# vincentfung13/MINE

Measured on AMD Instinct MI355X. Metric: train imgs/sec (whole node) RealEstate10K 384x256 N=64, higher is better.
Workload: dtype bf16; 1 GPU; model=monodepth2-resnet50-mpi, global_batch=4, seq_len=64, parallelism=dp1, img_h=256, img_w=384, n_planes=64

## Files before the change

mine_amd/ops/csrc/bindings.hip:

```cpp

#include <torch/extension.h>
#include <ATen/hip/HIPContext.h>
#include <hip/hip_runtime.h>

#include <vector>

extern "C" {
void mine_src_composite_fwd(const float*, const float*, const float*,
                            const float*, float*, float*, float*, int, int,
                            int, int, int, int, hipStream_t);
void mine_src_composite_bwd(const float*, const float*, const float*,
                            const float*, const float*, const float*,
                            const float*, float*, int, int, int, int, int,
                            int, hipStream_t);
void mine_tgt_composite_fwd(const float*, const float*, const float*,
                            const float*, const float*, float*, float*,
                            float*, int, int, int, int, int, int,
                            hipStream_t);
void mine_tgt_composite_bwd(const float*, const float*, const float*,
                            const float*, const float*, const float*,
                            const float*, const float*, float*, float*,
                            int, int, int, int, int, int, int, hipStream_t);
void mine_conv_igemm_fwd(const void*, const void*, const float*, void*,
                         float*, int64_t, int, int, int, int, int, int, int,
// ... 130 lines not shown
  const at::ScalarType t = dtype.value_or(at::kBFloat16);
  TORCH_CHECK(is_16bit(t), who, ": output dtype must be bf16 or fp16");
  return t;
}

std::vector<at::Tensor> src_composite_fwd(at::Tensor mpi, at::Tensor depths,
                                          at::Tensor kinv, at::Tensor img,
                                          bool bg_inf, bool alpha) {
  CHECK_IN(mpi); CHECK_IN(depths); CHECK_IN(kinv);
  TORCH_CHECK(mpi.dim() == 5 && mpi.size(4) == 4, "mpi must be (B,S,H,W,4)");
  const int B = mpi.size(0), S = mpi.size(1), H = mpi.size(2), W = mpi.size(3);
  TORCH_CHECK(S <= 192, "S too large for the LDS geometry stage");
  const bool blend = img.numel() > 0;
  if (blend) {
    CHECK_IN(img);
    TORCH_CHECK(img.sizes() == at::IntArrayRef({B, H, W, 3}),
                "img must be (B,H,W,3)");
  }
  auto rgb = at::empty({B, 3, H, W}, mpi.options());
  auto depth = at::empty({B, 1, H, W}, mpi.options());
  auto mpi_blend = blend ? at::empty_like(mpi) : at::empty({0}, mpi.options());
  mine_src_composite_fwd(mpi.data_ptr<float>(), depths.data_ptr<float>(),
                         kinv.data_ptr<float>(), optr(img),
                         rgb.data_ptr<float>(), depth.data_ptr<float>(),
                         blend ? mpi_blend.data_ptr<float>() : nullptr,
                         B, S, H, W, bg_inf ? 1 : 0, alpha ? 1 : 0,
                         stream());
  return {rgb, depth, mpi_blend};
}

at::Tensor src_composite_bwd(at::Tensor mpi, at::Tensor depths,
                             at::Tensor kinv, at::Tensor img, bool bg_inf,
                             bool alpha, at::Tensor g_rgb,
                             at::Tensor g_depth, at::Tensor g_blend) {
  CHECK_IN(mpi);
  const int B = mpi.size(0), S = mpi.size(1), H = mpi.size(2), W = mpi.size(3);
  auto grad_mpi = at::empty_like(mpi);
  mine_src_composite_bwd(mpi.data_ptr<float>(), depths.data_ptr<float>(),
                         kinv.data_ptr<float>(), optr(img), optr(g_rgb),
                         optr(g_depth), optr(g_blend),
                         grad_mpi.data_ptr<float>(), B, S, H, W,
                         bg_inf ? 1 : 0, alpha ? 1 : 0, stream());
  return grad_mpi;
}

std::vector<at::Tensor> tgt_composite_fwd(at::Tensor mpi, at::Tensor hinv,
                                          at::Tensor m, at::Tensor tvec,
                                          at::Tensor depths, bool bg_inf,
                                          bool alpha) {
  CHECK_IN(mpi); CHECK_IN(hinv); CHECK_IN(m); CHECK_IN(tvec); CHECK_IN(depths);
  TORCH_CHECK(mpi.dim() == 5 && mpi.size(4) == 4, "mpi must be (B,S,H,W,4)");
  const int B = mpi.size(0), S = mpi.size(1), H = mpi.size(2), W = mpi.size(3);
  TORCH_CHECK(S <= 192, "S too large for the LDS geometry stage");
  TORCH_CHECK(hinv.sizes() == at::IntArrayRef({B, S, 3, 3}));
  auto rgb = at::empty({B, 3, H, W}, mpi.options());
  auto depth = at::empty({B, 1, H, W}, mpi.options());
  auto mask = at::empty({B, 1, H, W}, mpi.options());
  mine_tgt_composite_fwd(mpi.data_ptr<float>(), hinv.data_ptr<float>(),
                         m.data_ptr<float>(), tvec.data_ptr<float>(),
                         depths.data_ptr<float>(), rgb.data_ptr<float>(),
                         depth.data_ptr<float>(), mask.data_ptr<float>(),
                         B, S, H, W, bg_inf ? 1 : 0, alpha ? 1 : 0,
                         stream());
  return {rgb, depth, mask};
}

at::Tensor tgt_composite_bwd(at::Tensor mpi, at::Tensor hinv, at::Tensor hfwd,
                             at::Tensor m, at::Tensor tvec, at::Tensor depths,
                             bool bg_inf, bool alpha, at::Tensor g_rgb,
                             at::Tensor g_depth, int64_t mode) {
  CHECK_IN(mpi);
  const int B = mpi.size(0), S = mpi.size(1), H = mpi.size(2), W = mpi.size(3);
  auto grad_mpi = at::zeros_like(mpi);
  at::Tensor payload;
  float* pay_ptr = nullptr;
  if (mode == 1) {
    TORCH_CHECK(hfwd.numel() == (int64_t)B * S * 9, "hfwd required in gather mode");
    payload = at::zeros_like(mpi);
    pay_ptr = payload.data_ptr<float>();
  }
  mine_tgt_composite_bwd(mpi.data_ptr<float>(), hinv.data_ptr<float>(),
                         mode == 1 ? hfwd.data_ptr<float>() : nullptr,
                         m.data_ptr<float>(), tvec.data_ptr<float>(),
                         depths.data_ptr<float>(), optr(g_rgb), optr(g_depth),
                         grad_mpi.data_ptr<float>(), pay_ptr, B, S, H, W,
                         bg_inf ? 1 : 0, (int)mode, alpha ? 1 : 0, stream());
  return grad_mpi;
}


at::Tensor eav2_fwd(at::Tensor disp, at::Tensor img, at::Tensor mean_d) {
  TORCH_CHECK(disp.is_cuda() && disp.is_contiguous() &&
              disp.scalar_type() == at::kFloat &&
              img.scalar_type() == at::kFloat);
  const int B = disp.size(0), H = disp.size(2), W = disp.size(3);
  auto out = at::zeros({2}, disp.options());
  mine_eav2_fwd(disp.data_ptr<float>(), img.data_ptr<float>(),
                mean_d.data_ptr<float>(), out.data_ptr<float>(), B, H, W,
                img.stride(0), img.stride(1), img.stride(2), img.stride(3),
                stream());
  return out;
}

at::Tensor eav2_bwd(at::Tensor disp, at::Tensor img, at::Tensor mean_d,
                    at::Tensor gl) {
  const int B = disp.size(0), H = disp.size(2), W = disp.size(3);
  auto g_d = at::empty({B, 1, H, W}, disp.options());
  auto Tb = at::zeros({B}, disp.options());
  auto grad = at::empty_like(disp);
  mine_eav2_bwd(disp.data_ptr<float>(), img.data_ptr<float>(),
                mean_d.data_ptr<float>(), g_d.data_ptr<float>(),
                Tb.data_ptr<float>(), gl.data_ptr<float>(),
                grad.data_ptr<float>(), B, H, W,
                img.stride(0), img.stride(1), img.stride(2), img.stride(3),
                stream());
  return grad;
}

at::Tensor pack_gather(at::Tensor w, at::Tensor lut,
                       c10::optional<at::ScalarType> dtype) {
  TORCH_CHECK(w.is_cuda() && w.is_contiguous() && lut.is_contiguous());
  TORCH_CHECK(lut.scalar_type() == at::kInt);
  TORCH_CHECK(w.scalar_type() == at::kFloat || is_16bit(w.scalar_type()),
              "pack_gather: weight must be f32, bf16 or fp16");
  const at::ScalarType ot = pack_dtype(dtype, "pack_gather");
  auto out = at::empty({lut.numel()}, w.options().dtype(ot));
  mine_pack_gather(w.data_ptr(), lut.data_ptr<int>(), out.data_ptr(),
                   lut.numel(), w_kind(w.scalar_type()),
                   ot == at::kHalf ? 1 : 0, stream());
  return out;
}
// ... 489 lines not shown
bool g_window_set = false;

void ensure_window() {
  if (g_window_set) return;
  double w[11], sum = 0.0;
  for (int i = 0; i < 11; ++i) {
    const double d = i - 5;
    w[i] = std::exp(-d * d / (2.0 * 1.5 * 1.5));
    sum += w[i];
  }
  float wf[11];
  for (int i = 0; i < 11; ++i) wf[i] = (float)(w[i] / sum);
  mine_ssim_set_window(wf);
  g_window_set = true;
}

std::vector<at::Tensor> ssim_fwd(at::Tensor img1, at::Tensor img2) {
  CHECK_IN(img1); CHECK_IN(img2);
  TORCH_CHECK(img1.dim() == 4 && img1.sizes() == img2.sizes());
  ensure_window();
  const int BC = img1.size(0) * img1.size(1);
  const int H = img1.size(2), W = img1.size(3);
  auto sum = at::zeros({1}, img1.options());
  mine_ssim_fwd(img1.data_ptr<float>(), img2.data_ptr<float>(),
                sum.data_ptr<float>(), BC, H, W, stream());
  return {(sum / (double)(BC * (int64_t)H * W)).squeeze(0)};
}

at::Tensor ssim_bwd(at::Tensor img1, at::Tensor img2, at::Tensor gscale) {
  CHECK_IN(img1); CHECK_IN(img2);
  ensure_window();
  const int BC = img1.size(0) * img1.size(1);
  const int H = img1.size(2), W = img1.size(3);
  auto F1 = at::empty_like(img1);
  auto F2 = at::empty_like(img1);
  auto F3 = at::empty_like(img1);
  auto grad1 = at::empty_like(img1);
  auto g = gscale.to(img1.options()).contiguous();
  mine_ssim_bwd(img1.data_ptr<float>(), img2.data_ptr<float>(),
                g.data_ptr<float>(), F1.data_ptr<float>(),
                F2.data_ptr<float>(), F3.data_ptr<float>(),
                grad1.data_ptr<float>(), BC, H, W, stream());
  return grad1;
}

}

PYBIND11_MODULE(TORCH_EXTENSION_NAME, mod) {
  mod.def("src_composite_fwd", &src_composite_fwd,
          "fused src-view MPI composite + RGB blend, forward");
  mod.def("src_composite_bwd", &src_composite_bwd);
  mod.def("tgt_composite_fwd", &tgt_composite_fwd,
          "fused plane-sweep warp + z-cull + composite, forward");
  mod.def("tgt_composite_bwd", &tgt_composite_bwd);
  mod.def("ssim_fwd", &ssim_fwd);
  mod.def("ssim_bwd", &ssim_bwd);
  mod.def("eav2_fwd", &eav2_fwd, "fused edge-aware smoothness v2 fwd");
  mod.def("eav2_bwd", &eav2_bwd, "fused edge-aware smoothness v2 bwd");
  namespace py = pybind11;
  mod.def("pack_gather", &pack_gather,
          "one-launch fragment pack through a device LUT", py::arg("w"),
          py::arg("lut"), py::arg("dtype") = py::none());
  mod.def("conv_igemm_fwd", &conv_igemm_fwd,
          "general igemm conv fwd / data-grad (coordinate-remapped)",
          py::arg("x_flat"), py::arg("wp"), py::arg("bias"), py::arg("M"),
          py::arg("P"), py::arg("Q"), py::arg("K"), py::arg("Hs"),
          py::arg("Ws"), py::arg("C"), py::arg("R"), py::arg("S"),
          py::arg("SA"), py::arg("SB"), py::arg("SD"), py::arg("SE"),
          py::arg("pad_mode"), py::arg("deterministic") = false);
  mod.def("conv_igemm_wrw", &conv_igemm_wrw,
          "general igemm conv weight-grad", py::arg("x_flat"),
          py::arg("gy_flat"), py::arg("M"), py::arg("P"), py::arg("Q"),
          py::arg("K"), py::arg("Hs"), py::arg("Ws"), py::arg("C"),
          py::arg("R"), py::arg("S"), py::arg("SA"), py::arg("SB"),
          py::arg("SD"), py::arg("SE"), py::arg("pad_mode"),
          py::arg("deterministic") = false);
  mod.def("upsample2x_fwd", &upsample2x_fwd,
          "nearest x2 upsample fwd, flat NHWC");
  mod.def("upsample2x_bwd", &upsample2x_bwd,
          "nearest x2 upsample bwd (4-child sum), flat NHWC");
  mod.def("reflect_pad_fwd", &reflect_pad_fwd,
          "gather reflection pad over logical (N,H,W,C)");
  mod.def("reflect_pad_bwd", &reflect_pad_bwd,
          "gather (atomic-free) reflection pad backward");
  mod.def("bn_stats", &bn_stats,
          "per-channel mean/invstd + running-stat update", py::arg("x"),
          py::arg("M"), py::arg("C"), py::arg("running_mean"),
          py::arg("running_var"), py::arg("eps"), py::arg("momentum"),
          py::arg("max_blocks") = 0, py::arg("deterministic") = false);
  mod.def("bn_sums", &bn_sums,
          "per-channel (sum, sumsq) only — for cross-rank SyncBN",
          py::arg("x"), py::arg("M"), py::arg("C"),
          py::arg("max_blocks") = 0, py::arg("deterministic") = false);
  mod.def("bn_finalize", &bn_finalize,
          "(sum, sumsq) -> mean/invstd + running-stat update");
  mod.def("bn_join_stats", &bn_join_stats,
          "x = (y_base + bias) + y_dec with its per-channel (sum, sumsq)",
          py::arg("y_dec"), py::arg("y_base"), py::arg("bias"), py::arg("B"),
          py::arg("S"), py::arg("HW"), py::arg("C"),
          py::arg("max_blocks") = 0, py::arg("deterministic") = false);
  mod.def("bn_act_fwd", &bn_act_fwd, "fused normalize + activation",
          py::arg("x"), py::arg("res"), py::arg("mean"), py::arg("invstd"),
          py::arg("gamma"), py::arg("beta"), py::arg("M"), py::arg("C"),
          py::arg("act"), py::arg("max_blocks") = 0);
  mod.def("bn_act_bwd", &bn_act_bwd,
          "fused BN+act backward -> dx, dres, dgamma, dbeta", py::arg("x"),
          py::arg("res"), py::arg("gy"), py::arg("mean"), py::arg("invstd"),
// ... 33 lines not shown
```

mine_amd/ops/csrc/render_kernels.hip:

```cpp

#include <hip/hip_runtime.h>
#include <cstdint>

#define DEV __device__ __forceinline__

namespace {

constexpr int kBlock = 256;
constexpr int kMaxS = 192;

struct float3x3 {
  float m[9];
  DEV float3 mul(float x, float y, float z) const {
    return make_float3(m[0] * x + m[1] * y + m[2] * z,
                       m[3] * x + m[4] * y + m[5] * z,
                       m[6] * x + m[7] * y + m[8] * z);
  }
};

DEV float clampf(float v, float lo, float hi) {
  return fminf(fmaxf(v, lo), hi);
}


// ... 203 lines not shown
      const float Af = (float)Ad;
      const PlaneTerm pt = src_plane_term<BLEND, BG_INF, ALPHA>(
          px, Af, I, gR, gD, d, delta, D, Wp, gC);
      const float u = ALPHA ? pt.t : (pt.t + 1e-6f);
      prefix += (double)pt.dA * Ad;
      const float dt = -Af * pt.e + (float)((TotalP - prefix) / (double)u);
      const float dsigma = (ALPHA ? -dt : dt * (-delta * pt.t)) + gCs;
      float4 g;
      if (BLEND) {
        const float oneA = 1.0f - Af;
        g = make_float4(oneA * pt.dcx, oneA * pt.dcy, oneA * pt.dcz, dsigma);
      } else {
        g = make_float4(pt.dcx, pt.dcy, pt.dcz, dsigma);
      }
      *reinterpret_cast<float4*>(grad_mpi + mpi_b + ((int64_t)s * HW + pix) * 4) = g;
      Ad *= (double)u;
      if (Ad < 1e-14) {
        for (int s2 = s + 1; s2 < S; ++s2) {
          const int64_t o = mpi_b + ((int64_t)s2 * HW + pix) * 4;
          float4 gt = make_float4(0.f, 0.f, 0.f, 0.f);
          if (BLEND && g_blend) {
            gt = *reinterpret_cast<const float4*>(g_blend + o);
          }
          *reinterpret_cast<float4*>(grad_mpi + o) = gt;
        }
        break;
      }
    }
  }
}


struct TapRef {
  int x0, x1, y0, y1;
  float wx, wy;
  bool interior;
};

DEV TapRef make_tap(float u, float v, int W, int H) {
  TapRef t;
  const float uc = clampf(u, 0.0f, (float)(W - 1));
  const float vc = clampf(v, 0.0f, (float)(H - 1));
  const float fx = floorf(uc), fy = floorf(vc);
  t.x0 = (int)fx;
  t.y0 = (int)fy;
  t.x1 = min(t.x0 + 1, W - 1);
  t.y1 = min(t.y0 + 1, H - 1);
  t.wx = uc - fx;
  t.wy = vc - fy;
  t.interior = (u == uc) && (v == vc);
  return t;
}

__device__ __attribute__((noinline)) float2
project_uv(const float* __restrict__ Hrow, int x, int y) {
  const float hx = Hrow[0] * x + Hrow[1] * y + Hrow[2];
  const float hy = Hrow[3] * x + Hrow[4] * y + Hrow[5];
  const float hz = Hrow[6] * x + Hrow[7] * y + Hrow[8];
  const float iz = 1.0f / hz;
  return make_float2(hx * iz, hy * iz);
}

DEV float4 bilinear4(const float* base, const TapRef& t, int W) {
  const float4 p00 = *reinterpret_cast<const float4*>(base + ((int64_t)t.y0 * W + t.x0) * 4);
  const float4 p01 = *reinterpret_cast<const float4*>(base + ((int64_t)t.y0 * W + t.x1) * 4);
  const float4 p10 = *reinterpret_cast<const float4*>(base + ((int64_t)t.y1 * W + t.x0) * 4);
  const float4 p11 = *reinterpret_cast<const float4*>(base + ((int64_t)t.y1 * W + t.x1) * 4);
  const float w00 = (1 - t.wx) * (1 - t.wy), w01 = t.wx * (1 - t.wy);
  const float w10 = (1 - t.wx) * t.wy, w11 = t.wx * t.wy;
  return make_float4(w00 * p00.x + w01 * p01.x + w10 * p10.x + w11 * p11.x,
                     w00 * p00.y + w01 * p01.y + w10 * p10.y + w11 * p11.y,
                     w00 * p00.z + w01 * p01.z + w10 * p10.z + w11 * p11.z,
                     w00 * p00.w + w01 * p01.w + w10 * p10.w + w11 * p11.w);
}

struct PlaneSample {
  float4 rgbs;
  float3 v;
  float inb;
};

__device__ __attribute__((noinline)) PlaneSample
sample_plane(const float* __restrict__ mpi_b, int s, int HW,
                             const float* __restrict__ s_geom, float d,
                             const float3x3& M, float3 tv,
                             int x, int y, int W, int H, TapRef* tap_out) {
  const float* Hrow = s_geom + s * 9;
  const float2 uv = project_uv(Hrow, x, y);
  const float u = uv.x, v = uv.y;

  PlaneSample ps;
  ps.inb = (u > -1.0f && u < (float)W && v > -1.0f && v < (float)H) ? 1.0f : 0.0f;

  const TapRef tap = make_tap(u, v, W, H);
  if (tap_out) *tap_out = tap;
  ps.rgbs = bilinear4(mpi_b + (int64_t)s * HW * 4, tap, W);

  const float ucl = clampf(u, 0.0f, (float)(W - 1));
  const float vcl = clampf(v, 0.0f, (float)(H - 1));
  const float3 r = M.mul(ucl, vcl, 1.0f);
  ps.v = make_float3(r.x * d + tv.x, r.y * d + tv.y, r.z * d + tv.z);
  if (ps.v.z < 0.0f) ps.rgbs.w = 0.0f;
  return ps;
}

template <bool BG_INF, bool ALPHA = false>
__global__ void __launch_bounds__(kBlock)
tgt_composite_fwd_kernel(const float* __restrict__ mpi,
                         const float* __restrict__ hinv,
                         const float* __restrict__ m_rki,
                         const float* __restrict__ tvec,
                         const float* __restrict__ depths,
                         float* __restrict__ rgb_out,
                         float* __restrict__ depth_out,
                         float* __restrict__ mask_out,
                         int B, int S, int H, int W) {
  __shared__ float s_geom[kMaxS * 9];
  __shared__ float s_depth[kMaxS];
  const int b = blockIdx.y;
  for (int i = threadIdx.x; i < S * 9; i += kBlock) s_geom[i] = hinv[(int64_t)b * S * 9 + i];
  for (int i = threadIdx.x; i < S; i += kBlock) s_depth[i] = depths[b * S + i];
  __syncthreads();

  float3x3 M;
#pragma unroll
  for (int i = 0; i < 9; ++i) M.m[i] = m_rki[b * 9 + i];
  const float3 tv = make_float3(tvec[b * 3], tvec[b * 3 + 1], tvec[b * 3 + 2]);

  const int HW = H * W;
  const float* mpi_b = mpi + (int64_t)b * S * HW * 4;
  for (int pix = blockIdx.x * kBlock + threadIdx.x; pix < HW;
       pix += gridDim.x * kBlock) {
    const int y = pix / W;
    const int x = pix - y * W;

    float A = 1.0f, Wsum = 0.0f, Nsum = 0.0f, mask = 0.0f;
    float3 R = make_float3(0.f, 0.f, 0.f);

    PlaneSample cur = sample_plane(mpi_b, 0, HW, s_geom, s_depth[0], M, tv,
                                   x, y, W, H, nullptr);
    mask += cur.inb;
    int s = 0;
    for (; s < S; ++s) {
      float delta;
      PlaneSample nxt;
      if (s + 1 < S) {
        nxt = sample_plane(mpi_b, s + 1, HW, s_geom, s_depth[s + 1], M, tv,
                           x, y, W, H, nullptr);
        mask += nxt.inb;
        const float dx = nxt.v.x - cur.v.x, dy = nxt.v.y - cur.v.y,
                    dz = nxt.v.z - cur.v.z;
        delta = sqrtf(dx * dx + dy * dy + dz * dz);
      } else {
        delta = 1e3f;
      }
      const float t = ALPHA ? (1.0f - cur.rgbs.w)
                            : __expf(-cur.rgbs.w * delta);
      const float w = A * (1.0f - t);
      R.x += w * cur.rgbs.x; R.y += w * cur.rgbs.y; R.z += w * cur.rgbs.z;
      Wsum += w;
      Nsum += w * cur.v.z;
      A *= ALPHA ? t : (t + 1e-6f);
      cur = nxt;
      if (A < 1e-14f) {
        ++s;
        break;
      }
    }
    for (int s2 = s + 1; s2 < S; ++s2) {
      const float* Hrow = s_geom + s2 * 9;
      const float hx = Hrow[0] * x + Hrow[1] * y + Hrow[2];
      const float hy = Hrow[3] * x + Hrow[4] * y + Hrow[5];
      const float hz = Hrow[6] * x + Hrow[7] * y + Hrow[8];
      const float iz = 1.0f / hz;
      const float u = hx * iz, v = hy * iz;
      mask += (u > -1.0f && u < (float)W && v > -1.0f && v < (float)H)
                  ? 1.0f : 0.0f;
    }
    const float D = ALPHA ? Nsum
                          : (BG_INF ? (Nsum + 1000.0f * (1.0f - Wsum))
                                    : (Nsum / (Wsum + 1e-5f)));
    rgb_out[((int64_t)b * 3 + 0) * HW + pix] = R.x;
    rgb_out[((int64_t)b * 3 + 1) * HW + pix] = R.y;
    rgb_out[((int64_t)b * 3 + 2) * HW + pix] = R.z;
    depth_out[(int64_t)b * HW + pix] = D;
    mask_out[(int64_t)b * HW + pix] = mask;
  }
}

DEV void scatter4(float* base, const TapRef& t, int W, float4 g) {
  const float w00 = (1 - t.wx) * (1 - t.wy), w01 = t.wx * (1 - t.wy);
  const float w10 = (1 - t.wx) * t.wy, w11 = t.wx * t.wy;
  float* p00 = base + ((int64_t)t.y0 * W + t.x0) * 4;
  float* p01 = base + ((int64_t)t.y0 * W + t.x1) * 4;
  float* p10 = base + ((int64_t)t.y1 * W + t.x0) * 4;
  float* p11 = base + ((int64_t)t.y1 * W + t.x1) * 4;
#define SC(P, WGT)                                  \
  if (WGT != 0.0f) {                                \
    atomicAdd(P + 0, WGT * g.x);                    \
    atomicAdd(P + 1, WGT * g.y);                    \
    atomicAdd(P + 2, WGT * g.z);                    \
    atomicAdd(P + 3, WGT * g.w);                    \
  }
  SC(p00, w00) SC(p01, w01) SC(p10, w10) SC(p11, w11)
#undef SC
}

__device__ __attribute__((noinline)) float plane_delta(float3 a, float3 b) {
  const float dx = b.x - a.x, dy = b.y - a.y, dz = b.z - a.z;
  return sqrtf(dx * dx + dy * dy + dz * dz);
}

struct TgtTerm {
  float t, r, cr, cv, cw;
};

template <bool ALPHA>
__device__ __attribute__((noinline)) TgtTerm
tgt_plane_terms(float4 rgbs, float vz, float delta, float3 gR) {
  TgtTerm o;
  o.t = ALPHA ? (1.0f - rgbs.w) : __expf(-rgbs.w * delta);
  o.r = rgbs.x * gR.x + rgbs.y * gR.y + rgbs.z * gR.z;
  const float omt = 1.0f - o.t;
  o.cr = omt * o.r;
  o.cv = omt * vz;
  o.cw = omt;
  return o;
}

template <bool BG_INF, bool GATHER, bool ALPHA = false>
__global__ void __launch_bounds__(kBlock)
tgt_composite_bwd_kernel(const float* __restrict__ mpi,
                         const float* __restrict__ hinv,
                         const float* __restrict__ m_rki,
                         const float* __restrict__ tvec,
                         const float* __restrict__ depths,
                         const float* __restrict__ g_rgb,
                         const float* __restrict__ g_depth,
                         float* __restrict__ grad_mpi,
                         float* __restrict__ payload,
                         int B, int S, int H, int W) {
  __shared__ float s_geom[kMaxS * 9];
  __shared__ float s_depth[kMaxS];
  const int b = blockIdx.y;
  for (int i = threadIdx.x; i < S * 9; i += kBlock) s_geom[i] = hinv[(int64_t)b * S * 9 + i];
  for (int i = threadIdx.x; i < S; i += kBlock) s_depth[i] = depths[b * S + i];
  __syncthreads();

  float3x3 M;
#pragma unroll
  for (int i = 0; i < 9; ++i) M.m[i] = m_rki[b * 9 + i];
  const float3 tv = make_float3(tvec[b * 3], tvec[b * 3 + 1], tvec[b * 3 + 2]);

  const int HW = H * W;
  const float* mpi_b = mpi + (int64_t)b * S * HW * 4;
  float* gm_b = grad_mpi + (int64_t)b * S * HW * 4;
  for (int pix = blockIdx.x * kBlock + threadIdx.x; pix < HW;
       pix += gridDim.x * kBlock) {
    const int y = pix / W;
    const int x = pix - y * W;

    float3 gR = make_float3(0.f, 0.f, 0.f);
    if (g_rgb) {
      gR.x = g_rgb[((int64_t)b * 3 + 0) * HW + pix];
      gR.y = g_rgb[((int64_t)b * 3 + 1) * HW + pix];
      gR.z = g_rgb[((int64_t)b * 3 + 2) * HW + pix];
    }
    const float gD = g_depth ? g_depth[(int64_t)b * HW + pix] : 0.0f;

    float A = 1.0f, Wsum = 0.0f, Nsum = 0.0f;
    double TaR = 0.0, TaV = 0.0, TaW = 0.0;
    double Ad = 1.0;
    PlaneSample cur = sample_plane(mpi_b, 0, HW, s_geom, s_depth[0], M, tv,
                                   x, y, W, H, nullptr);
    for (int s = 0; s < S; ++s) {
      float delta;
      PlaneSample nxt;
      if (s + 1 < S) {
        nxt = sample_plane(mpi_b, s + 1, HW, s_geom, s_depth[s + 1], M, tv,
                           x, y, W, H, nullptr);
        delta = plane_delta(cur.v, nxt.v);
      } else {
        delta = 1e3f;
      }
      const TgtTerm tt = tgt_plane_terms<ALPHA>(cur.rgbs, cur.v.z, delta,
                                                gR);
      const float w = A * (1.0f - tt.t);
      Wsum += w;
      Nsum += w * cur.v.z;
      TaR += (double)tt.cr * Ad;
      TaV += (double)tt.cv * Ad;
      TaW += (double)tt.cw * Ad;
      A *= ALPHA ? tt.t : (tt.t + 1e-6f);
      Ad *= (double)(ALPHA ? tt.t : (tt.t + 1e-6f));
      cur = nxt;
      if (Ad < 1e-14) break;
    }
    const float Wp = Wsum + 1e-5f;
    const float D = BG_INF ? (Nsum + 1000.0f * (1.0f - Wsum)) : (Nsum / Wp);
    const float qv = ALPHA ? gD : (BG_INF ? gD : gD / Wp);
    const float qc = ALPHA ? 0.0f
                           : (BG_INF ? (-1000.0f * gD) : (-gD / Wp * D));

    double prR = 0.0, prV = 0.0, prW = 0.0;
    Ad = 1.0;
    TapRef tap;
    cur = sample_plane(mpi_b, 0, HW, s_geom, s_depth[0], M, tv, x, y, W, H,
                       &tap);
    for (int s = 0; s < S; ++s) {
      float delta;
      PlaneSample nxt;
      TapRef ntap;
      if (s + 1 < S) {
        nxt = sample_plane(mpi_b, s + 1, HW, s_geom, s_depth[s + 1], M, tv,
                           x, y, W, H, &ntap);
        delta = plane_delta(cur.v, nxt.v);
      } else {
        delta = 1e3f;
      }
      const TgtTerm tt = tgt_plane_terms<ALPHA>(cur.rgbs, cur.v.z, delta,
                                                gR);
      const float t = tt.t;
      const float u = ALPHA ? t : (t + 1e-6f);
      const float Af = (float)Ad;
      const float w = Af * (1.0f - t);
      prR += (double)tt.cr * Ad;
      prV += (double)tt.cv * Ad;
      prW += (double)tt.cw * Ad;
      const double suffix = (TaR - prR) + (double)qv * (TaV - prV) +
                            (double)qc * (TaW - prW);
      const float e = tt.r + qv * cur.v.z + qc;
      const float dt = -Af * e + (float)(suffix / (double)u);
      const float dsigma = (cur.v.z < 0.0f)
          ? 0.0f : (ALPHA ? -dt : dt * (-delta * t));
      const float4 g = make_float4(w * gR.x, w * gR.y, w * gR.z, dsigma);
      if (GATHER && tap.interior) {
        *reinterpret_cast<float4*>(
            payload + ((int64_t)b * S + s) * HW * 4 + (int64_t)pix * 4) = g;
      } else {
        scatter4(gm_b + (int64_t)s * HW * 4, tap, W, g);
      }
      Ad *= (double)u;
      cur = nxt;
      tap = ntap;
      if (Ad < 1e-14) break;
    }
  }
}


constexpr int GT = 32;

__global__ void __launch_bounds__(kBlock)
tgt_gather_kernel(const float* __restrict__ payload,
                  const float* __restrict__ hinv,
                  const float* __restrict__ hfwd,
                  float* __restrict__ grad_mpi,
                  int B, int S, int H, int W, int tiles_x) {
  __shared__ float s_acc[GT * GT * 4];
  __shared__ float s_Hi[9];
  __shared__ float s_Hf[9];
  const int tile = blockIdx.x;
  const int s = blockIdx.y;
  const int b = blockIdx.z;
  const int tx0 = (tile % tiles_x) * GT;
  const int ty0 = (tile / tiles_x) * GT;
  const int tid = threadIdx.x;

  for (int i = tid; i < GT * GT * 4; i += kBlock) s_acc[i] = 0.0f;
  if (tid < 9) {
    s_Hi[tid] = hinv[((int64_t)b * S + s) * 9 + tid];
    s_Hf[tid] = hfwd[((int64_t)b * S + s) * 9 + tid];
  }
  __syncthreads();

  float bx0 = 0.f, by0 = 0.f, bx1 = (float)(W - 1), by1 = (float)(H - 1);
  {
    const float cx[2] = {(float)tx0 - 1.25f, (float)(tx0 + GT) + 0.25f};
    const float cy[2] = {(float)ty0 - 1.25f, (float)(ty0 + GT) + 0.25f};
    float mnx = 1e30f, mny = 1e30f, mxx = -1e30f, mxy = -1e30f;
    bool ok = true;
#pragma unroll
    for (int ci = 0; ci < 4; ++ci) {
      const float x = cx[ci & 1], y = cy[ci >> 1];
      const float qz = s_Hf[6] * x + s_Hf[7] * y + s_Hf[8];
      const float qx = (s_Hf[0] * x + s_Hf[1] * y + s_Hf[2]) / qz;
      const float qy = (s_Hf[3] * x + s_Hf[4] * y + s_Hf[5]) / qz;
      ok = ok && (qz > 1e-8f) && isfinite(qx) && isfinite(qy);
      mnx = fminf(mnx, qx); mny = fminf(mny, qy);
      mxx = fmaxf(mxx, qx); mxy = fmaxf(mxy, qy);
    }
    if (ok) {
      bx0 = fmaxf(0.f, floorf(mnx - 1.0f));
      by0 = fmaxf(0.f, floorf(mny - 1.0f));
      bx1 = fminf((float)(W - 1), ceilf(mxx + 1.0f));
      by1 = fminf((float)(H - 1), ceilf(mxy + 1.0f));
    }
  }
  const int px0 = (int)bx0, py0 = (int)by0;
  const int bw = (int)bx1 - px0 + 1, bh = (int)by1 - py0 + 1;
  const int HW = H * W;
  const float* pay_b = payload + ((int64_t)b * S + s) * HW * 4;

  if (bw > 0 && bh > 0) {
    for (int i = tid; i < bw * bh; i += kBlock) {
      const int px = px0 + i % bw;
      const int py = py0 + i / bw;
      const float4 g = *reinterpret_cast<const float4*>(
          pay_b + ((int64_t)py * W + px) * 4);
      if (g.x == 0.f && g.y == 0.f && g.z == 0.f && g.w == 0.f) continue;
      const float2 uv = project_uv(s_Hi, px, py);
      const TapRef t = make_tap(uv.x, uv.y, W, H);
      if (!t.interior) continue;
      const float w00 = (1 - t.wx) * (1 - t.wy), w01 = t.wx * (1 - t.wy);
      const float w10 = (1 - t.wx) * t.wy, w11 = t.wx * t.wy;
#define GSC(QX, QY, WGT)                                              \
      if (WGT != 0.0f && (QX) >= tx0 && (QX) < tx0 + GT &&            \
          (QY) >= ty0 && (QY) < ty0 + GT) {                           \
        float* a = s_acc + (((QY) - ty0) * GT + ((QX) - tx0)) * 4;    \
        atomicAdd(a + 0, WGT * g.x);                                  \
        atomicAdd(a + 1, WGT * g.y);                                  \
        atomicAdd(a + 2, WGT * g.z);                                  \
        atomicAdd(a + 3, WGT * g.w);                                  \
      }
      GSC(t.x0, t.y0, w00) GSC(t.x1, t.y0, w01)
      GSC(t.x0, t.y1, w10) GSC(t.x1, t.y1, w11)
#undef GSC
    }
  }
  __syncthreads();

  float* gm = grad_mpi + ((int64_t)b * S + s) * HW * 4;
  for (int i = tid; i < GT * GT; i += kBlock) {
    const int qx = tx0 + i % GT;
    const int qy = ty0 + i / GT;
    if (qx >= W || qy >= H) continue;
    const float4 a = *reinterpret_cast<const float4*>(s_acc + i * 4);
    if (a.x == 0.f && a.y == 0.f && a.z == 0.f && a.w == 0.f) continue;
    float4* dst = reinterpret_cast<float4*>(gm + ((int64_t)qy * W + qx) * 4);
    float4 cur = *dst;
    cur.x += a.x; cur.y += a.y; cur.z += a.z; cur.w += a.w;
    *dst = cur;
  }
}

inline int grid_x(int HW) {
  int g = (HW + kBlock - 1) / kBlock;
  return g < 4096 ? g : 4096;
}

}


#define DISPATCH_BOOL(VAL, NAME, ...)          \
  if (VAL) {                                   \
    constexpr bool NAME = true;                \
    __VA_ARGS__;                               \
  } else {                                     \
    constexpr bool NAME = false;               \
    __VA_ARGS__;                               \
  }

extern "C" {

void mine_src_composite_fwd(const float* mpi, const float* depths,
                            const float* kinv, const float* img,
                            float* rgb_out, float* depth_out, float* mpi_blend,
                            int B, int S, int H, int W, int bg_inf, int alpha,
                            hipStream_t stream) {
  dim3 grid(grid_x(H * W), B);
  const bool blend = img != nullptr;
  if (alpha) {
    hipLaunchKernelGGL((src_composite_fwd_kernel<false, false, true>), grid,
                       dim3(kBlock), 0, stream, mpi, depths, kinv, nullptr,
                       rgb_out, depth_out, mpi_blend, B, S, H, W);
    return;
  }
  DISPATCH_BOOL(blend, BLEND, {
    DISPATCH_BOOL(bg_inf, BG, {
      hipLaunchKernelGGL((src_composite_fwd_kernel<BLEND, BG>), grid,
                         dim3(kBlock), 0, stream, mpi, depths, kinv, img,
                         rgb_out, depth_out, mpi_blend, B, S, H, W);
    })
  })
}

void mine_src_composite_bwd(const float* mpi, const float* depths,
                            const float* kinv, const float* img,
                            const float* g_rgb, const float* g_depth,
                            const float* g_blend, float* grad_mpi,
                            int B, int S, int H, int W, int bg_inf, int alpha,
                            hipStream_t stream) {
  dim3 grid(grid_x(H * W), B);
  const bool blend = img != nullptr;
  if (alpha) {
    hipLaunchKernelGGL((src_composite_bwd_kernel<false, false, true>), grid,
                       dim3(kBlock), 0, stream, mpi, depths, kinv, nullptr,
                       g_rgb, g_depth, nullptr, grad_mpi, B, S, H, W);
    return;
  }
  DISPATCH_BOOL(blend, BLEND, {
    DISPATCH_BOOL(bg_inf, BG, {
      hipLaunchKernelGGL((src_composite_bwd_kernel<BLEND, BG>), grid,
                         dim3(kBlock), 0, stream, mpi, depths, kinv, img,
                         g_rgb, g_depth, g_blend, grad_mpi, B, S, H, W);
    })
  })
}

void mine_tgt_composite_fwd(const float* mpi, const float* hinv,
                            const float* m_rki, const float* tvec,
                            const float* depths, float* rgb_out,
                            float* depth_out, float* mask_out,
                            int B, int S, int H, int W, int bg_inf, int alpha,
                            hipStream_t stream) {
  dim3 grid(grid_x(H * W), B);
  if (alpha) {
    hipLaunchKernelGGL((tgt_composite_fwd_kernel<false, true>), grid,
                       dim3(kBlock), 0, stream, mpi, hinv, m_rki, tvec,
                       depths, rgb_out, depth_out, mask_out, B, S, H, W);
    return;
  }
  DISPATCH_BOOL(bg_inf, BG, {
    hipLaunchKernelGGL((tgt_composite_fwd_kernel<BG>), grid, dim3(kBlock), 0,
                       stream, mpi, hinv, m_rki, tvec, depths, rgb_out,
                       depth_out, mask_out, B, S, H, W);
  })
}

void mine_tgt_composite_bwd(const float* mpi, const float* hinv,
                            const float* hfwd, const float* m_rki,
                            const float* tvec, const float* depths,
                            const float* g_rgb, const float* g_depth,
                            float* grad_mpi, float* payload,
                            int B, int S, int H, int W, int bg_inf, int mode,
                            int alpha, hipStream_t stream) {
  dim3 grid(grid_x(H * W), B);
#define TGT_BWD_BODY(BGv, ALv)                                                if (mode == 1) {                                                              hipLaunchKernelGGL((tgt_composite_bwd_kernel<BGv, true, ALv>), grid,                           dim3(kBlock), 0, stream, mpi, hinv, m_rki, tvec,                            depths, g_rgb, g_depth, grad_mpi, payload,                                  B, S, H, W);                                             const int tiles_x = (W + GT - 1) / GT;                                      const int tiles_y = (H + GT - 1) / GT;                                      dim3 ggrid(tiles_x * tiles_y, S, B);                                        hipLaunchKernelGGL(tgt_gather_kernel, ggrid, dim3(kBlock), 0, stream,                          payload, hinv, hfwd, grad_mpi, B, S, H, W, tiles_x);   } else {                                                                      hipLaunchKernelGGL((tgt_composite_bwd_kernel<BGv, false, ALv>), grid,                          dim3(kBlock), 0, stream, mpi, hinv, m_rki, tvec,                            depths, g_rgb, g_depth, grad_mpi, nullptr,                                  B, S, H, W);                                           }
  if (alpha) {
    TGT_BWD_BODY(false, true)
    return;
  }
  DISPATCH_BOOL(bg_inf, BG, { TGT_BWD_BODY(BG, false) })
#undef TGT_BWD_BODY
}

}
```

Baseline: 82.91 imgs/sec.

## Rework target-composite backward gather: wave-level non-atomic LDS accumulation, planar LDS, reusable workspace

Rewrites the gather kernel to run one 64-lane wavefront per tile. Each wave processes rows in chunks of four and checks with ballots and shuffles whether its bilinear taps are monotone and free of duplicates. When they are, it accumulates into a planar LDS layout with plain adds, ordered by parity, instead of LDS atomics. The backward scatter kernel now writes zeros into the payload explicitly, including planes after early termination, so the payload can use empty_like or a caller-supplied workspace instead of zeros_like. Helpers are inlined with explicit fma, pointer offsets become 32-bit, and a double divide is replaced by a float divide. The costs are more complex, correctness-sensitive conflict detection, small numeric differences, and a 64-thread block that may lower occupancy efficiency.

```diff
diff --git a/mine_amd/ops/csrc/bindings.hip b/mine_amd/ops/csrc/bindings.hip
--- a/mine_amd/ops/csrc/bindings.hip
+++ b/mine_amd/ops/csrc/bindings.hip
@@ -206,6 +206,8 @@
   TORCH_CHECK(mpi.dim() == 5 && mpi.size(4) == 4, "mpi must be (B,S,H,W,4)");
   const int B = mpi.size(0), S = mpi.size(1), H = mpi.size(2), W = mpi.size(3);
   TORCH_CHECK(S <= 192, "S too large for the LDS geometry stage");
+  TORCH_CHECK((int64_t)H * W * 4 < (int64_t(1) << 31),
+              "one plane must stay below 2^31 floats (32-bit tap offsets)");
   TORCH_CHECK(hinv.sizes() == at::IntArrayRef({B, S, 3, 3}));
   auto rgb = at::empty({B, 3, H, W}, mpi.options());
   auto depth = at::empty({B, 1, H, W}, mpi.options());
@@ -222,15 +224,26 @@
 at::Tensor tgt_composite_bwd(at::Tensor mpi, at::Tensor hinv, at::Tensor hfwd,
                              at::Tensor m, at::Tensor tvec, at::Tensor depths,
                              bool bg_inf, bool alpha, at::Tensor g_rgb,
-                             at::Tensor g_depth, int64_t mode) {
+                             at::Tensor g_depth, int64_t mode,
+                             c10::optional<at::Tensor> workspace) {
   CHECK_IN(mpi);
   const int B = mpi.size(0), S = mpi.size(1), H = mpi.size(2), W = mpi.size(3);
+  TORCH_CHECK((int64_t)H * W * 4 < (int64_t(1) << 31),
+              "one plane must stay below 2^31 floats (32-bit tap offsets)");
   auto grad_mpi = at::zeros_like(mpi);
   at::Tensor payload;
   float* pay_ptr = nullptr;
   if (mode == 1) {
     TORCH_CHECK(hfwd.numel() == (int64_t)B * S * 9, "hfwd required in gather mode");
-    payload = at::zeros_like(mpi);
+    if (workspace.has_value()) {
+      payload = *workspace;
+      CHECK_IN(payload);
+      TORCH_CHECK(payload.numel() == mpi.numel() &&
+                  payload.device() == mpi.device(),
+                  "workspace must match mpi in size and device");
+    } else {
+      payload = at::empty_like(mpi);
+    }
     pay_ptr = payload.data_ptr<float>();
   }
   mine_tgt_composite_bwd(mpi.data_ptr<float>(), hinv.data_ptr<float>(),
@@ -826,7 +839,12 @@
   mod.def("src_composite_bwd", &src_composite_bwd);
   mod.def("tgt_composite_fwd", &tgt_composite_fwd,
           "fused plane-sweep warp + z-cull + composite, forward");
-  mod.def("tgt_composite_bwd", &tgt_composite_bwd);
+  mod.def("tgt_composite_bwd", &tgt_composite_bwd, pybind11::arg("mpi"),
+          pybind11::arg("hinv"), pybind11::arg("hfwd"), pybind11::arg("m"),
+          pybind11::arg("tvec"), pybind11::arg("depths"),
+          pybind11::arg("bg_inf"), pybind11::arg("alpha"),
+          pybind11::arg("g_rgb"), pybind11::arg("g_depth"),
+          pybind11::arg("mode"), pybind11::arg("workspace") = pybind11::none());
   mod.def("ssim_fwd", &ssim_fwd);
   mod.def("ssim_bwd", &ssim_bwd);
   mod.def("eav2_fwd", &eav2_fwd, "fused edge-aware smoothness v2 fwd");
diff --git a/mine_amd/ops/csrc/render_kernels.hip b/mine_amd/ops/csrc/render_kernels.hip
--- a/mine_amd/ops/csrc/render_kernels.hip
+++ b/mine_amd/ops/csrc/render_kernels.hip
@@ -279,56 +279,71 @@
   return t;
 }
 
-__device__ __attribute__((noinline)) float2
-project_uv(const float* __restrict__ Hrow, int x, int y) {
-  const float hx = Hrow[0] * x + Hrow[1] * y + Hrow[2];
-  const float hy = Hrow[3] * x + Hrow[4] * y + Hrow[5];
-  const float hz = Hrow[6] * x + Hrow[7] * y + Hrow[8];
+DEV float2 project_uv(const float* Hrow, int x, int y) {
+#pragma clang fp contract(off)
+  const float fx = (float)x, fy = (float)y;
+  const float hx = fmaf(Hrow[0], fx, fmaf(Hrow[1], fy, Hrow[2]));
+  const float hy = fmaf(Hrow[3], fx, fmaf(Hrow[4], fy, Hrow[5]));
+  const float hz = fmaf(Hrow[6], fx, fmaf(Hrow[7], fy, Hrow[8]));
   const float iz = 1.0f / hz;
   return make_float2(hx * iz, hy * iz);
 }
 
+DEV bool uv_interior(float u, float v, int W, int H) {
+  return (u == clampf(u, 0.0f, (float)(W - 1))) &&
+         (v == clampf(v, 0.0f, (float)(H - 1)));
+}
+
 DEV float4 bilinear4(const float* base, const TapRef& t, int W) {
-  const float4 p00 = *reinterpret_cast<const float4*>(base + ((int64_t)t.y0 * W + t.x0) * 4);
-  const float4 p01 = *reinterpret_cast<const float4*>(base + ((int64_t)t.y0 * W + t.x1) * 4);
-  const float4 p10 = *reinterpret_cast<const float4*>(base + ((int64_t)t.y1 * W + t.x0) * 4);
-  const float4 p11 = *reinterpret_cast<const float4*>(base + ((int64_t)t.y1 * W + t.x1) * 4);
+#pragma clang fp contract(off)
+  const float4 p00 = *reinterpret_cast<const float4*>(base + (unsigned)(t.y0 * W + t.x0) * 4u);
+  const float4 p01 = *reinterpret_cast<const float4*>(base + (unsigned)(t.y0 * W + t.x1) * 4u);
+  const float4 p10 = *reinterpret_cast<const float4*>(base + (unsigned)(t.y1 * W + t.x0) * 4u);
+  const float4 p11 = *reinterpret_cast<const float4*>(base + (unsigned)(t.y1 * W + t.x1) * 4u);
   const float w00 = (1 - t.wx) * (1 - t.wy), w01 = t.wx * (1 - t.wy);
   const float w10 = (1 - t.wx) * t.wy, w11 = t.wx * t.wy;
-  return make_float4(w00 * p00.x + w01 * p01.x + w10 * p10.x + w11 * p11.x,
-                     w00 * p00.y + w01 * p01.y + w10 * p10.y + w11 * p11.y,
-                     w00 * p00.z + w01 * p01.z + w10 * p10.z + w11 * p11.z,
-                     w00 * p00.w + w01 * p01.w + w10 * p10.w + w11 * p11.w);
+#define BL(C) fmaf(w11, p11.C, fmaf(w10, p10.C, fmaf(w01, p01.C, w00 * p00.C)))
+  return make_float4(BL(x), BL(y), BL(z), BL(w));
+#undef BL
 }
 
 struct PlaneSample {
   float4 rgbs;
   float3 v;
   float inb;
+  float pu, pv;
 };
 
-__device__ __attribute__((noinline)) PlaneSample
-sample_plane(const float* __restrict__ mpi_b, int s, int HW,
-                             const float* __restrict__ s_geom, float d,
+DEV PlaneSample sample_plane(const float* mpi_b, int s, int HW,
+                             const float* s_geom, float d,
                              const float3x3& M, float3 tv,
-                             int x, int y, int W, int H, TapRef* tap_out) {
-  const float* Hrow = s_geom + s * 9;
-  const float2 uv = project_uv(Hrow, x, y);
+                             int x, int y, int W, int H) {
+#pragma clang fp contract(off)
+  const float2 uv = project_uv(s_geom + s * 9, x, y);
   const float u = uv.x, v = uv.y;
 
   PlaneSample ps;
+  ps.pu = u;
+  ps.pv = v;
   ps.inb = (u > -1.0f && u < (float)W && v > -1.0f && v < (float)H) ? 1.0f : 0.0f;
 
   const TapRef tap = make_tap(u, v, W, H);
-  if (tap_out) *tap_out = tap;
   ps.rgbs = bilinear4(mpi_b + (int64_t)s * HW * 4, tap, W);
 
   const float ucl = clampf(u, 0.0f, (float)(W - 1));
   const float vcl = clampf(v, 0.0f, (float)(H - 1));
-  const float3 r = M.mul(ucl, vcl, 1.0f);
-  ps.v = make_float3(r.x * d + tv.x, r.y * d + tv.y, r.z * d + tv.z);
+  const float rx = fmaf(M.m[0], ucl, fmaf(M.m[1], vcl, M.m[2]));
+  const float ry = fmaf(M.m[3], ucl, fmaf(M.m[4], vcl, M.m[5]));
+  const float rz = fmaf(M.m[6], ucl, fmaf(M.m[7], vcl, M.m[8]));
+  ps.v = make_float3(fmaf(rx, d, tv.x), fmaf(ry, d, tv.y), fmaf(rz, d, tv.z));
   if (ps.v.z < 0.0f) ps.rgbs.w = 0.0f;
   return ps;
+}
+
+DEV float plane_delta(float3 a, float3 b) {
+#pragma clang fp contract(off)
+  const float dx = b.x - a.x, dy = b.y - a.y, dz = b.z - a.z;
+  return sqrtf(fmaf(dz, dz, fmaf(dy, dy, dx * dx)));
 }
 
 template <bool BG_INF, bool ALPHA = false>
@@ -365,7 +380,7 @@
     float3 R = make_float3(0.f, 0.f, 0.f);
 
     PlaneSample cur = sample_plane(mpi_b, 0, HW, s_geom, s_depth[0], M, tv,
-                                   x, y, W, H, nullptr);
+                                   x, y, W, H);
     mask += cur.inb;
     int s = 0;
     for (; s < S; ++s) {
@@ -373,11 +388,9 @@
       PlaneSample nxt;
       if (s + 1 < S) {
         nxt = sample_plane(mpi_b, s + 1, HW, s_geom, s_depth[s + 1], M, tv,
-                           x, y, W, H, nullptr);
+                           x, y, W, H);
         mask += nxt.inb;
-        const float dx = nxt.v.x - cur.v.x, dy = nxt.v.y - cur.v.y,
-                    dz = nxt.v.z - cur.v.z;
-        delta = sqrtf(dx * dx + dy * dy + dz * dz);
+        delta = plane_delta(cur.v, nxt.v);
       } else {
         delta = 1e3f;
       }
@@ -395,12 +408,8 @@
       }
     }
     for (int s2 = s + 1; s2 < S; ++s2) {
-      const float* Hrow = s_geom + s2 * 9;
-      const float hx = Hrow[0] * x + Hrow[1] * y + Hrow[2];
-      const float hy = Hrow[3] * x + Hrow[4] * y + Hrow[5];
-      const float hz = Hrow[6] * x + Hrow[7] * y + Hrow[8];
-      const float iz = 1.0f / hz;
-      const float u = hx * iz, v = hy * iz;
+      const float2 uv = project_uv(s_geom + s2 * 9, x, y);
+      const float u = uv.x, v = uv.y;
       mask += (u > -1.0f && u < (float)W && v > -1.0f && v < (float)H)
                   ? 1.0f : 0.0f;
     }
@@ -418,10 +427,10 @@
 DEV void scatter4(float* base, const TapRef& t, int W, float4 g) {
   const float w00 = (1 - t.wx) * (1 - t.wy), w01 = t.wx * (1 - t.wy);
   const float w10 = (1 - t.wx) * t.wy, w11 = t.wx * t.wy;
-  float* p00 = base + ((int64_t)t.y0 * W + t.x0) * 4;
-  float* p01 = base + ((int64_t)t.y0 * W + t.x1) * 4;
-  float* p10 = base + ((int64_t)t.y1 * W + t.x0) * 4;
-  float* p11 = base + ((int64_t)t.y1 * W + t.x1) * 4;
+  float* p00 = base + (unsigned)(t.y0 * W + t.x0) * 4u;
+  float* p01 = base + (unsigned)(t.y0 * W + t.x1) * 4u;
+  float* p10 = base + (unsigned)(t.y1 * W + t.x0) * 4u;
+  float* p11 = base + (unsigned)(t.y1 * W + t.x1) * 4u;
 #define SC(P, WGT)                                  \
   if (WGT != 0.0f) {                                \
     atomicAdd(P + 0, WGT * g.x);                    \
@@ -433,21 +442,16 @@
 #undef SC
 }
 
-__device__ __attribute__((noinline)) float plane_delta(float3 a, float3 b) {
-  const float dx = b.x - a.x, dy = b.y - a.y, dz = b.z - a.z;
-  return sqrtf(dx * dx + dy * dy + dz * dz);
-}
-
 struct TgtTerm {
   float t, r, cr, cv, cw;
 };
 
 template <bool ALPHA>
-__device__ __attribute__((noinline)) TgtTerm
-tgt_plane_terms(float4 rgbs, float vz, float delta, float3 gR) {
+DEV TgtTerm tgt_plane_terms(float4 rgbs, float vz, float delta, float3 gR) {
+#pragma clang fp contract(off)
   TgtTerm o;
   o.t = ALPHA ? (1.0f - rgbs.w) : __expf(-rgbs.w * delta);
-  o.r = rgbs.x * gR.x + rgbs.y * gR.y + rgbs.z * gR.z;
+  o.r = fmaf(rgbs.z, gR.z, fmaf(rgbs.y, gR.y, rgbs.x * gR.x));
   const float omt = 1.0f - o.t;
   o.cr = omt * o.r;
   o.cv = omt * vz;
@@ -499,13 +503,13 @@
     double TaR = 0.0, TaV = 0.0, TaW = 0.0;
     double Ad = 1.0;
     PlaneSample cur = sample_plane(mpi_b, 0, HW, s_geom, s_depth[0], M, tv,
-                                   x, y, W, H, nullptr);
+                                   x, y, W, H);
     for (int s = 0; s < S; ++s) {
       float delta;
       PlaneSample nxt;
       if (s + 1 < S) {
         nxt = sample_plane(mpi_b, s + 1, HW, s_geom, s_depth[s + 1], M, tv,
-                           x, y, W, H, nullptr);
+                           x, y, W, H);
         delta = plane_delta(cur.v, nxt.v);
       } else {
         delta = 1e3f;
@@ -531,16 +535,16 @@
 
     double prR = 0.0, prV = 0.0, prW = 0.0;
     Ad = 1.0;
-    TapRef tap;
-    cur = sample_plane(mpi_b, 0, HW, s_geom, s_depth[0], M, tv, x, y, W, H,
-                       &tap);
-    for (int s = 0; s < S; ++s) {
+    float* pay_b = GATHER ? payload + (int64_t)b * S * HW * 4 : nullptr;
+    const float4 zero4 = make_float4(0.f, 0.f, 0.f, 0.f);
+    cur = sample_plane(mpi_b, 0, HW, s_geom, s_depth[0], M, tv, x, y, W, H);
+    int s = 0;
+    for (; s < S; ++s) {
       float delta;
       PlaneSample nxt;
-      TapRef ntap;
       if (s + 1 < S) {
         nxt = sample_plane(mpi_b, s + 1, HW, s_geom, s_depth[s + 1], M, tv,
-                           x, y, W, H, &ntap);
+                           x, y, W, H);
         delta = plane_delta(cur.v, nxt.v);
       } else {
         delta = 1e3f;
@@ -557,34 +561,51 @@
       const double suffix = (TaR - prR) + (double)qv * (TaV - prV) +
                             (double)qc * (TaW - prW);
       const float e = tt.r + qv * cur.v.z + qc;
-      const float dt = -Af * e + (float)(suffix / (double)u);
+      const float dt = -Af * e + (float)suffix / u;
       const float dsigma = (cur.v.z < 0.0f)
           ? 0.0f : (ALPHA ? -dt : dt * (-delta * t));
       const float4 g = make_float4(w * gR.x, w * gR.y, w * gR.z, dsigma);
-      if (GATHER && tap.interior) {
-        *reinterpret_cast<float4*>(
-            payload + ((int64_t)b * S + s) * HW * 4 + (int64_t)pix * 4) = g;
-      } else {
-        scatter4(gm_b + (int64_t)s * HW * 4, tap, W, g);
+      const bool interior = GATHER && uv_interior(cur.pu, cur.pv, W, H);
+      if (GATHER) {
+        *reinterpret_cast<float4*>(pay_b + (int64_t)s * HW * 4 +
+                                   (unsigned)pix * 4u) =
+            make_float4(interior ? g.x : 0.f, interior ? g.y : 0.f,
+                        interior ? g.z : 0.f, interior ? g.w : 0.f);
+      }
+      if (!interior) {
+        scatter4(gm_b + (int64_t)s * HW * 4,
+                 make_tap(cur.pu, cur.pv, W, H), W, g);
       }
       Ad *= (double)u;
       cur = nxt;
-      tap = ntap;
       if (Ad < 1e-14) break;
     }
-  }
-}
-
+    if (GATHER) {
+      for (int s2 = s + 1; s2 < S; ++s2) {
+        *reinterpret_cast<float4*>(pay_b + (int64_t)s2 * HW * 4 +
+                                   (unsigned)pix * 4u) = zero4;
+      }
+    }
+  }
+}
+
+
+DEV void lds_add(float* p, float v) {
+#pragma clang fp contract(off)
+  *p = *p + v;
+}
 
 constexpr int GT = 32;
-
-__global__ void __launch_bounds__(kBlock)
+constexpr int kGBlock = 64;
+constexpr int kGRows = 4;
+
+__global__ void __launch_bounds__(kGBlock)
 tgt_gather_kernel(const float* __restrict__ payload,
                   const float* __restrict__ hinv,
                   const float* __restrict__ hfwd,
                   float* __restrict__ grad_mpi,
                   int B, int S, int H, int W, int tiles_x) {
-  __shared__ float s_acc[GT * GT * 4];
+  __shared__ float s_acc[4 * GT * GT];
   __shared__ float s_Hi[9];
   __shared__ float s_Hf[9];
   const int tile = blockIdx.x;
@@ -594,7 +615,7 @@
   const int ty0 = (tile / tiles_x) * GT;
   const int tid = threadIdx.x;
 
-  for (int i = tid; i < GT * GT * 4; i += kBlock) s_acc[i] = 0.0f;
+  for (int i = tid; i < GT * GT * 4; i += kGBlock) s_acc[i] = 0.0f;
   if (tid < 9) {
     s_Hi[tid] = hinv[((int64_t)b * S + s) * 9 + tid];
     s_Hf[tid] = hfwd[((int64_t)b * S + s) * 9 + tid];
@@ -630,39 +651,98 @@
   const float* pay_b = payload + ((int64_t)b * S + s) * HW * 4;
 
   if (bw > 0 && bh > 0) {
-    for (int i = tid; i < bw * bh; i += kBlock) {
-      const int px = px0 + i % bw;
-      const int py = py0 + i / bw;
-      const float4 g = *reinterpret_cast<const float4*>(
-          pay_b + ((int64_t)py * W + px) * 4);
-      if (g.x == 0.f && g.y == 0.f && g.z == 0.f && g.w == 0.f) continue;
-      const float2 uv = project_uv(s_Hi, px, py);
-      const TapRef t = make_tap(uv.x, uv.y, W, H);
-      if (!t.interior) continue;
-      const float w00 = (1 - t.wx) * (1 - t.wy), w01 = t.wx * (1 - t.wy);
-      const float w10 = (1 - t.wx) * t.wy, w11 = t.wx * t.wy;
-#define GSC(QX, QY, WGT)                                              \
-      if (WGT != 0.0f && (QX) >= tx0 && (QX) < tx0 + GT &&            \
-          (QY) >= ty0 && (QY) < ty0 + GT) {                           \
-        float* a = s_acc + (((QY) - ty0) * GT + ((QX) - tx0)) * 4;    \
-        atomicAdd(a + 0, WGT * g.x);                                  \
-        atomicAdd(a + 1, WGT * g.y);                                  \
-        atomicAdd(a + 2, WGT * g.z);                                  \
-        atomicAdd(a + 3, WGT * g.w);                                  \
-      }
-      GSC(t.x0, t.y0, w00) GSC(t.x1, t.y0, w01)
-      GSC(t.x0, t.y1, w10) GSC(t.x1, t.y1, w11)
+    const int lane = tid;
+    for (int r0 = 0; r0 < bh; r0 += kGRows) {
+      for (int c0 = 0; c0 < bw; c0 += 64) {
+        const int cx = c0 + lane;
+        const bool in_chunk = cx < bw;
+        const int px = px0 + cx;
+        float4 g[kGRows];
+#pragma unroll
+        for (int k = 0; k < kGRows; ++k) {
+          g[k] = make_float4(0.f, 0.f, 0.f, 0.f);
+          if (in_chunk && r0 + k < bh) {
+            g[k] = *reinterpret_cast<const float4*>(
+                pay_b + (unsigned)((py0 + r0 + k) * W + px) * 4u);
+          }
+        }
+#pragma unroll
+        for (int k = 0; k < kGRows; ++k) {
+          if (r0 + k >= bh) break;
+          const float4 gk = g[k];
+          const int py = py0 + r0 + k;
+          const float2 uv = project_uv(s_Hi, px, py);
+          const TapRef t = make_tap(uv.x, uv.y, W, H);
+          const bool adds = in_chunk &&
+              !(gk.x == 0.f && gk.y == 0.f && gk.z == 0.f && gk.w == 0.f) &&
+              uv_interior(uv.x, uv.y, W, H);
+          if (!__any(adds)) continue;
+
+          const int x0l = __shfl_up(t.x0, 1), y0l = __shfl_up(t.y0, 1);
+          const bool has_l = in_chunk && lane >= 1;
+          const bool mono_x = __all(!has_l || t.x0 >= x0l) ||
+                              __all(!has_l || t.x0 <= x0l);
+          const bool mono_y = __all(!has_l || t.y0 >= y0l) ||
+                              __all(!has_l || t.y0 <= y0l);
+          const unsigned long long starts =
+              __ballot(!(has_l && t.x0 == x0l && t.y0 == y0l));
+          const unsigned long long addm = __ballot(adds);
+          const unsigned long long upto = (2ull << lane) - 1ull;
+          const int start = 63 - __clzll((long long)(starts & upto));
+          const unsigned long long left =
+              (upto >> 1) & ~((1ull << start) - 1ull);
+          const unsigned long long par = (lane & 1) ? 0xAAAAAAAAAAAAAAAAull
+                                                    : 0x5555555555555555ull;
+          const bool no_dup = __all(!(adds && (addm & left & par) != 0ull));
+          const bool plain = mono_x && mono_y && no_dup;
+
+          const float w00 = (1 - t.wx) * (1 - t.wy), w01 = t.wx * (1 - t.wy);
+          const float w10 = (1 - t.wx) * t.wy, w11 = t.wx * t.wy;
+#define GSC(ADD, QX, QY, WGT)                                         \
+          if (WGT != 0.0f && (QX) >= tx0 && (QX) < tx0 + GT &&        \
+              (QY) >= ty0 && (QY) < ty0 + GT) {                       \
+            float* a = s_acc + ((QY) - ty0) * GT + ((QX) - tx0);      \
+            ADD(a + 0 * GT * GT, WGT * gk.x);                         \
+            ADD(a + 1 * GT * GT, WGT * gk.y);                         \
+            ADD(a + 2 * GT * GT, WGT * gk.z);                         \
+            ADD(a + 3 * GT * GT, WGT * gk.w);                         \
+          }
+#define GSC4(ADD)                                                     \
+          GSC(ADD, t.x0, t.y0, w00) TAP_ORDER                         \
+          GSC(ADD, t.x1, t.y0, w01) TAP_ORDER                         \
+          GSC(ADD, t.x0, t.y1, w10) TAP_ORDER                         \
+          GSC(ADD, t.x1, t.y1, w11)
+#define TAP_ORDER                                                     \
+          __builtin_amdgcn_fence(__ATOMIC_ACQ_REL, "wavefront");      \
+          __builtin_amdgcn_wave_barrier();
+#define ADD_PLAIN(P, V) lds_add((P), (V))
+#define ADD_ATOMIC(P, V) atomicAdd((P), (V))
+          if (plain) {
+            if (adds && (lane & 1) == 0) { GSC4(ADD_PLAIN) }
+            TAP_ORDER
+            if (adds && (lane & 1) == 1) { GSC4(ADD_PLAIN) }
+          } else if (adds) {
+            GSC4(ADD_ATOMIC)
+          }
+#undef ADD_ATOMIC
+#undef ADD_PLAIN
+#undef TAP_ORDER
+#undef GSC4
 #undef GSC
+        }
+      }
     }
   }
   __syncthreads();
 
   float* gm = grad_mpi + ((int64_t)b * S + s) * HW * 4;
-  for (int i = tid; i < GT * GT; i += kBlock) {
-    const int qx = tx0 + i % GT;
+  for (int i = tid; i < GT * GT; i += kGBlock) {
+    const int qx = tx0 + (i & (GT - 1));
     const int qy = ty0 + i / GT;
     if (qx >= W || qy >= H) continue;
-    const float4 a = *reinterpret_cast<const float4*>(s_acc + i * 4);
+    const float4 a = make_float4(s_acc[i], s_acc[GT * GT + i],
+                                 s_acc[2 * GT * GT + i],
+                                 s_acc[3 * GT * GT + i]);
     if (a.x == 0.f && a.y == 0.f && a.z == 0.f && a.w == 0.f) continue;
     float4* dst = reinterpret_cast<float4*>(gm + ((int64_t)qy * W + qx) * 4);
     float4 cur = *dst;
@@ -763,7 +843,7 @@
                             int B, int S, int H, int W, int bg_inf, int mode,
                             int alpha, hipStream_t stream) {
   dim3 grid(grid_x(H * W), B);
-#define TGT_BWD_BODY(BGv, ALv)                                                if (mode == 1) {                                                              hipLaunchKernelGGL((tgt_composite_bwd_kernel<BGv, true, ALv>), grid,                           dim3(kBlock), 0, stream, mpi, hinv, m_rki, tvec,                            depths, g_rgb, g_depth, grad_mpi, payload,                                  B, S, H, W);                                             const int tiles_x = (W + GT - 1) / GT;                                      const int tiles_y = (H + GT - 1) / GT;                                      dim3 ggrid(tiles_x * tiles_y, S, B);                                        hipLaunchKernelGGL(tgt_gather_kernel, ggrid, dim3(kBlock), 0, stream,                          payload, hinv, hfwd, grad_mpi, B, S, H, W, tiles_x);   } else {                                                                      hipLaunchKernelGGL((tgt_composite_bwd_kernel<BGv, false, ALv>), grid,                          dim3(kBlock), 0, stream, mpi, hinv, m_rki, tvec,                            depths, g_rgb, g_depth, grad_mpi, nullptr,                                  B, S, H, W);                                           }
+#define TGT_BWD_BODY(BGv, ALv)                                                if (mode == 1) {                                                              hipLaunchKernelGGL((tgt_composite_bwd_kernel<BGv, true, ALv>), grid,                           dim3(kBlock), 0, stream, mpi, hinv, m_rki, tvec,                            depths, g_rgb, g_depth, grad_mpi, payload,                                  B, S, H, W);                                             const int tiles_x = (W + GT - 1) / GT;                                      const int tiles_y = (H + GT - 1) / GT;                                      dim3 ggrid(tiles_x * tiles_y, S, B);                                        hipLaunchKernelGGL(tgt_gather_kernel, ggrid, dim3(kGBlock), 0, stream,                          payload, hinv, hfwd, grad_mpi, B, S, H, W, tiles_x);   } else {                                                                      hipLaunchKernelGGL((tgt_composite_bwd_kernel<BGv, false, ALv>), grid,                          dim3(kBlock), 0, stream, mpi, hinv, m_rki, tvec,                            depths, g_rgb, g_depth, grad_mpi, nullptr,                                  B, S, H, W);                                           }
   if (alpha) {
     TGT_BWD_BODY(false, true)
     return;
```

New measurement: 87.79 imgs/sec (median of 6 runs). +5.9%, better.
